# andrewcsmith/soundsym

Measured on AMD Instinct MI355X. Metric: segment-pairs/sec (DTW cost+argmin), higher is better.
Workload: dtype f32

## Files before the change

soundsym_amd/csrc/dtw_filter.hip:

```cpp
#include "ssym_internal.hpp"
#include "dtw_filter_kernel.hpp"
#include "dtw_filter_wg_kernel.hpp"
#include "dtw_filter_wg2_kernel.hpp"
#include "dtw_filter_pk_kernel.hpp"
#include "dtw_filter_sp_kernel.hpp"
#include "dtw_band_kernel.hpp"

#include <algorithm>
#include <atomic>
#include <cmath>
#include <cstdlib>

namespace ssym {

static std::atomic<unsigned long long> g_filter_wg_launches{0};
static std::atomic<unsigned long long> g_filter_wg2_launches{0};
static std::atomic<bool> g_filter_wg2{true};

int filter_pieces(int dim)
{
    static const bool k48 = ssym_knob("SSYM_FILTER_K48") != nullptr;
    return dim > kFilterMaxDim2 ? 1 : (k48 ? 2 : 3);
}

__global__ void build_filter_records_kernel(const double *__restrict__ raw, const uint64_t *__restrict__ off,
                                            const uint32_t *__restrict__ perm, uint32_t n, uint32_t dim,
                                            uint32_t dimUse, uint32_t frames_pad, int is_source,
                                            int lead, int pieces, double scale, _Float16 *__restrict__ rec,
                                            unsigned *__restrict__ resid)
{
    const uint32_t s = blockIdx.y;
    const uint32_t seg = perm[s];
    const uint32_t slot = blockIdx.x * blockDim.x + threadIdx.x;
    if (slot >= frames_pad)
        return;
    _Float16 out[kFilterRecHalfs];
#pragma unroll
    for (int i = 0; i < kFilterRecHalfs; ++i)
        out[i] = (_Float16)0.0f;
    const uint32_t nf = seg < n ? (uint32_t)(off[seg + 1] - off[seg]) : 0u;
    const uint32_t first = lead < 0 ? frames_pad - nf : (uint32_t)lead;
    const bool real = slot >= first && slot < first + nf;
    const uint32_t f = slot - first;
    const int nbase = pieces == 3 ? 28 : (pieces == 2 ? 3 : 1) * (int)dimUse;
    const int npieces = pieces == 3 ? 2 : 3;
    if (!real && is_source)
        out[filter_slot_offset(nbase)] = (_Float16)__builtin_inff();
    if (real) {
        const double *p = raw + (off[seg] + f) * dim;
        double nrm = 0.0, res2 = 0.0;
        for (uint32_t e = 0; e < dimUse; ++e) {
            const double v = p[e] * scale;
            const _Float16 h1 = (_Float16)v;
            const bool two = pieces == 2 || (pieces == 3 && (is_source || e < 2));
            const _Float16 h2 = two ? (_Float16)(v - (double)h1) : (_Float16)0.0f;
            const double vh = (double)h1 + (double)h2;
            nrm += vh * vh;
            res2 += (v - vh) * (v - vh);
            const _Float16 m1 = (_Float16)(-2.0f * (float)h1), m2 = (_Float16)(-2.0f * (float)h2);
            if (pieces == 2) {
                out[filter_slot_offset(3 * e + 0)] = is_source ? m1 : h1;
                out[filter_slot_offset(3 * e + 1)] = is_source ? m1 : h2;
                out[filter_slot_offset(3 * e + 2)] = is_source ? m2 : h1;
            } else if (pieces == 3) {
                out[filter_slot_offset(2 * e + 0)] = is_source ? m1 : h1;
                out[filter_slot_offset(2 * e + 1)] = is_source ? m2 : h1;
                if (e < 2)
                    out[filter_slot_offset(26 + e)] = is_source ? m1 : h2;
            } else {
                out[filter_slot_offset(e)] = is_source ? m1 : h1;
            }
        }
        const float r = __double2float_ru(sqrt(res2) / scale * 1.0000001);
        if (r > 0.0f)
            atomicMax(&resid[s], __float_as_uint(r));
        const _Float16 p1 = (_Float16)nrm;
        const _Float16 p2 = (_Float16)(nrm - (double)p1);
        const _Float16 p3 = (_Float16)(nrm - (double)p1 - (double)p2);
        const int mine = nbase + (is_source ? 0 : npieces), other = nbase + (is_source ? npieces : 0);
        out[filter_slot_offset(mine + 0)] = p1;
        out[filter_slot_offset(mine + 1)] = p2;
        out[filter_slot_offset(other + 0)] = (_Float16)1.0f;
        out[filter_slot_offset(other + 1)] = (_Float16)1.0f;
        if (npieces == 3) {
            out[filter_slot_offset(mine + 2)] = p3;
            out[filter_slot_offset(other + 2)] = (_Float16)1.0f;
        }
    }
    if (is_source) {
        _Float16 *dst = rec + ((size_t)s * frames_pad + slot) * kFilterRecHalfs;
#pragma unroll
        for (int i = 0; i < kFilterRecHalfs; ++i)
            dst[i] = out[i];
    } else {
#pragma unroll
        for (int h = 0; h < 2; ++h)
#pragma unroll
            for (int m = 0; m < kFilterKM; ++m) {
                _Float16 *dst = rec + tgt_rec_offset(s, frames_pad, slot, m, h);
#pragma unroll
// ... 7 lines not shown
{
    const uint32_t kb = (uint32_t)(2 * radius + 1 + 15) / 16 * 16;
    return std::max<uint32_t>(radius + src.max_frames, std::max<uint32_t>(tgt.max_frames, 1) + kb) + 1;
}
static size_t band_lds_bytes(int radius, const SegmentSet &src, const SegmentSet &tgt)
{
    return ((size_t)2 * band_slots(radius, src, tgt) * kFilterRecHalfs + kBandImagePad) * sizeof(_Float16);
}

bool filter_band_as_bound(const ssym_ctx *ctx, const SegmentSet &src, const SegmentSet &tgt)
{
    if (ctx->band < 0)
        return false;
    return 2 * ctx->band + 1 > 6 * 16 || band_lds_bytes(ctx->band, src, tgt) > 160 * 1024 - 64;
}

bool filter_supported(const ssym_ctx *ctx, const SegmentSet &src, const SegmentSet &tgt)
{
    if (src.light || tgt.light)
        return false;
    if (src.dim != tgt.dim)
        return false;
    if ((ctx->band < 0 || filter_band_as_bound(ctx, src, tgt)) && filter_shape((int)src.max_frames).nt == 0)
        return false;
    if (!std::isfinite(src.max_abs) || !std::isfinite(tgt.max_abs))
        return false;
    if (!std::isfinite(src.max_sqnorm_all) || !std::isfinite(tgt.max_sqnorm_all))
        return false;
    return src.n > 0 && tgt.n > 0;
}

static double common_scale(const SegmentSet &src, const SegmentSet &tgt)
{
    const double m = std::max(src.max_abs, tgt.max_abs);
    if (!(m > 0.0))
        return 1.0;
    int e = 0;
    (void)std::frexp(m, &e);
    e = std::min(std::max(6 - e, -100), 100);
    const double sq = std::max(src.max_sqnorm_all, tgt.max_sqnorm_all);
    while (e > -200 && sq * std::ldexp(1.0, 2 * e) * 1.01 >= 65000.0)
        --e;
    const double ideal = std::ldexp(1.0, e);
    if (src.rec && src.rec_scale > 0.0 && src.rec_scale <= ideal && src.rec_scale * 16.0 >= ideal)
        return src.rec_scale;
    return ideal;
}

static int32_t ensure_records(ssym_ctx *ctx, const SegmentSet &set, double scale, uint32_t slots, int lead)
{
    const size_t bytes = (size_t)set.n_pad * slots * kFilterRecHalfs * sizeof(_Float16);
    if (set.rec && set.rec_scale == scale && set.rec_bytes == bytes && set.rec_slots == slots &&
        set.rec_lead == lead)
        return SSYM_OK;
    if (set.rec && set.rec_bytes != bytes) {
        dev_free(ctx, set.rec);
        set.rec = nullptr;
    }
    if (!set.rec) {
        int32_t rca = dev_alloc(ctx, &set.rec, bytes);
        if (rca != SSYM_OK)
            return rca;
    }
    set.rec_bytes = bytes;
    dim3 grid((slots + 63) / 64, set.n_pad);
    const int dimUse = filter_dim_used((int)set.dim);
    unsigned *resid = (unsigned *)(set.max_sqnorm + 2 * (size_t)set.n_pad);
    SSYM_HIP_CHECK(ctx, hipMemsetAsync(resid, 0, sizeof(unsigned) * set.n_pad, ctx->stream));
    build_filter_records_kernel<<<grid, 64, 0, ctx->stream>>>(set.raw, set.off, set.perm, set.n, set.dim,
                                                              (uint32_t)dimUse, slots, set.is_source ? 1 : 0, lead,
                                                              filter_pieces(dimUse), scale,
                                                              (_Float16 *)set.rec, resid);
    SSYM_HIP_CHECK(ctx, hipGetLastError());
    set.rec_scale = scale;
    set.rec_slots = slots;
    set.rec_lead = lead;
    return SSYM_OK;
}

static FilterKnobs read_filter_knobs()
{
    FilterKnobs k;
    g_filter_wg2.store(true, std::memory_order_relaxed);
    if (!ssym_knob("SSYM_TEST_HOOKS"))
        return k;
    auto num = [](const char *name, int unset) {
        const char *v = ssym_knob(name);
        return v ? atoi(v) : unset;
    };
    k.pk = num("SSYM_FILTER_PK", 0) != 0;
    k.sp = num("SSYM_FILTER_SP", 1) != 0;
    const int mp = num("SSYM_SP_MULTIPAIR", 1);
    k.spMultipair = mp == 0 || mp == 2 ? mp : 1;
    k.spPairBlock = ssym_knob("SSYM_SP_PAIRBLOCK") ? std::max(num("SSYM_SP_PAIRBLOCK", 0), 0) : -1;
    k.wg = num("SSYM_FILTER_WG", k.wg) != 0;
    g_filter_wg2.store(num("SSYM_FILTER_WG2", 1) != 0, std::memory_order_relaxed);
    k.skip0 = num("SSYM_FILTER_SKIP0", 1) != 0;
    k.nt8 = ssym_knob("SSYM_FILTER_NT8") != nullptr;
    k.oneLaunch = ssym_knob("SSYM_FILTER_ONE_LAUNCH") != nullptr;
    k.longClasses = num("SSYM_FILTER_LONG_CLASSES", 1) != 0;
    k.pruneNt = num("SSYM_PRUNE_NT", 0);
    return k;
}

static const std::vector<uint32_t> &plan_lens(const SegmentSet &set, uint32_t group)
{
    if (set.plan_lens.size() != set.n_pad / group) {
        set.plan_lens.assign(set.n_pad / group, 0u);
        for (uint32_t slot = 0; slot < set.n; ++slot) {
            const uint32_t s = set.h_perm[slot];
            uint32_t &m = set.plan_lens[slot / group];
            m = std::max(m, (uint32_t)(set.h_off[s + 1] - set.h_off[s]));
        }
    }
    return set.plan_lens;
}

struct FilterCall {
    hipStream_t st;
    const SegmentSet &src, &tgt;
    bool sq;
    int ku;
    float outScale;
    float *handoff;
    unsigned *taskCtr;
    float *cmat;
    const float *abandon;
    unsigned long long *colCtr;
    const uint32_t *candSlot;
    bool wg2;
};

template <int NT, bool SQ, int KU>
static bool run_kernel(const FilterCall &c, const FilterLaunch &l)
{
    constexpr int OCC = NT == 1 ? 3 : NT == 8 ? 1 : 2;
    const dim3 grid(l.grid), block(64 * kFilterWavesPerBlock);
    const _Float16 *srec = (const _Float16 *)c.src.rec, *trec = (const _Float16 *)c.tgt.rec;
    const int rowsPad = (int)c.src.frames_pad, colsPad = (int)c.tgt.frames_pad, tgtPad = (int)c.tgt.n_pad;
    const int nSrcPairs = l.hi - l.lo, nTasks = nSrcPairs * (tgtPad / 32);
    unsigned *ctr = c.taskCtr + l.ctrSet * 8 * kTaskCtrStride;
    switch (l.kind) {
    case FilterKernel::Mp:
        if constexpr (NT == 1) {
            dtw_filter_sp_kernel<KU == 2 ? 3 : 2, SQ, 2, KU, kSpRowBlock, true><<<grid, block, 0, c.st>>>(
                srec, trec, c.src.len, c.tgt.len, rowsPad, colsPad, tgtPad, l.taskPairs, nSrcPairs, l.taskChunk, c.outScale,
                ctr, c.cmat, l.origin, l.lo, l.pairBlock);
            return true;
        }
        return false;
    case FilterKernel::Sp:
        if constexpr (NT <= 3 && (KU == 2 || NT <= 2)) {
            constexpr int OCCSP = (NT == 1 && KU == 2) ? 3 : (NT == 2 && KU == 2) ? SSYM_SP_OCC_NT2 : 2;
            dtw_filter_sp_kernel<NT, SQ, OCCSP, KU, kSpRowBlock><<<grid, block, 0, c.st>>>(
                srec, trec, c.src.len, c.tgt.len, rowsPad, colsPad, tgtPad, nSrcPairs, nTasks, l.taskChunk, c.outScale, ctr,
                c.cmat, l.origin, l.lo, l.pairBlock);
            return true;
        }
        return false;
    case FilterKernel::GenericSkip0:
        if constexpr (NT == 3 || NT == 4) {
            dtw_filter_kernel<NT, SQ, OCC, false, KU, true><<<grid, block, 0, c.st>>>(
                srec, trec, c.src.len, c.tgt.len, rowsPad, l.passes, colsPad, tgtPad, nSrcPairs, nTasks, l.taskChunk,
                c.outScale, c.handoff, ctr, c.cmat, nullptr, nullptr, nullptr, l.origin, l.lo);
            return true;
        }
        return false;
    case FilterKernel::Wg:
        if constexpr (NT == 4) {
            if (l.passes == 2 && c.wg2) {
                dtw_filter_wg2_kernel<SQ, KU><<<grid, block, 0, c.st>>>(
                    srec, trec, c.src.len, c.tgt.len, rowsPad, colsPad, tgtPad, nSrcPairs / 4, l.taskChunk, c.outScale, ctr,
                    c.cmat, l.origin, l.lo);
                g_filter_wg_launches.fetch_add(1, std::memory_order_relaxed);
                g_filter_wg2_launches.fetch_add(1, std::memory_order_relaxed);
                return true;
            }
            dtw_filter_wg_kernel<SQ, KU><<<grid, block, 0, c.st>>>(
                srec, trec, c.src.len, c.tgt.len, rowsPad, l.passes, colsPad, tgtPad, nSrcPairs / 4, l.taskChunk, c.outScale,
                c.handoff, ctr, c.cmat, l.origin, l.lo);
            g_filter_wg_launches.fetch_add(1, std::memory_order_relaxed);
            return true;
        }
        return false;
    case FilterKernel::Pk:
        if constexpr (NT == 4) {
            dtw_filter_pk_kernel<SQ, KU><<<grid, block, 0, c.st>>>(
                srec, trec, c.src.len, c.tgt.len, rowsPad, l.passes, colsPad, tgtPad, nSrcPairs, nTasks, l.taskChunk,
                c.outScale, c.handoff, ctr, c.cmat, l.origin, l.lo);
            return true;
        }
        return false;
    case FilterKernel::GenericPrune:
        dtw_filter_kernel<NT, SQ, OCC, true, KU><<<grid, block, 0, c.st>>>(
            srec, trec, c.src.len, c.tgt.len, rowsPad, l.passes, colsPad, tgtPad, nSrcPairs, nTasks, l.taskChunk, c.outScale,
            c.handoff, ctr, c.cmat, c.abandon, c.colCtr, c.candSlot, l.origin, l.lo);
        return true;
    case FilterKernel::Generic:
        dtw_filter_kernel<NT, SQ, OCC, false, KU><<<grid, block, 0, c.st>>>(
            srec, trec, c.src.len, c.tgt.len, rowsPad, l.passes, colsPad, tgtPad, nSrcPairs, nTasks, l.taskChunk, c.outScale,
            c.handoff, ctr, c.cmat, nullptr, nullptr, nullptr, l.origin, l.lo);
        return true;
    }
    return false;
}

template <int NT>
static bool run_tiles(const FilterCall &c, const FilterLaunch &l)
{
    if (c.sq)
        return c.ku == 2 ? run_kernel<NT, true, 2>(c, l) : run_kernel<NT, true, 3>(c, l);
    return c.ku == 2 ? run_kernel<NT, false, 2>(c, l) : run_kernel<NT, false, 3>(c, l);
}

static bool run_launch(const FilterCall &c, const FilterLaunch &l)
{
    switch (l.nt) {
    case 1: return run_tiles<1>(c, l);
    case 2: return run_tiles<2>(c, l);
    case 3: return run_tiles<3>(c, l);
    case 4: return run_tiles<4>(c, l);
    case 8: return run_tiles<8>(c, l);
    }
    return false;
}

template <int NTB, int WB, int OCC, bool SQ, int LASTN, bool PRUNE>
static int32_t launch_band_cfg2(ssym_ctx *ctx, const SegmentSet &src, const SegmentSet &tgt, uint32_t slots,
                                size_t lds, float outScale, float *cmat, const float *abandon,
                                unsigned long long *colCtr, const uint32_t *candSlot)
{
    const int nTgtBlocks = (int)tgt.n_pad / (32 * WB);
    const int nTasks = ((int)src.n_pad / 2) * nTgtBlocks;
    const int grid = std::max(1, std::min(ctx->num_cus, nTasks));
    int32_t rc = ensure(ctx, ctx->handoff, 8 * sizeof(unsigned));
    if (rc != SSYM_OK)
        return rc;
    unsigned *taskCtr = (unsigned *)ctx->handoff.ptr;
    rc = zero_words(ctx, taskCtr, sizeof(unsigned));
    if (rc != SSYM_OK)
        return rc;
    const bool two = filter_mfmas(filter_pieces(filter_dim_used((int)src.dim)), filter_dim_used((int)src.dim)) == 2;
    auto kern = two ? dtw_band_kernel<NTB, WB, OCC, SQ, LASTN, PRUNE, 2> : dtw_band_kernel<NTB, WB, OCC, SQ, LASTN, PRUNE, 3>;
#ifdef SSYM_BAND_PAIRCOLS_BUILD
    if constexpr (!PRUNE && LASTN == 1 && NTB >= 4 && OCC == 2) {
        const char *pc = ssym_knob("SSYM_BAND_PAIRCOLS");
        if (pc && atoi(pc) != 0)
            kern = two ? dtw_band_kernel<NTB, WB, OCC, SQ, LASTN, PRUNE, 2, true> : dtw_band_kernel<NTB, WB, OCC, SQ, LASTN, PRUNE, 3, true>;
    }
#endif
    if (lds > 64 * 1024)
        SSYM_HIP_CHECK(ctx, hipFuncSetAttribute((const void *)kern, hipFuncAttributeMaxDynamicSharedMemorySize, (int)lds));
    kern<<<dim3(grid), 64 * WB, lds, ctx->stream>>>(
// ... 40 lines not shown
        return rc;
    rc = ensure_records(ctx, tgt, scale, tgt.frames_pad, 0);
    if (rc != SSYM_OK)
        return rc;
    const bool sq = ctx->squared != 0;
    const float outScale = (float)(sq ? 1.0 / (scale * scale) : 1.0 / scale);
    const int ntb = (2 * ctx->band + 1 + 15) / 16;
#define SSYM_BCASE(N_)                                                                                  \
    case N_:                                                                                            \
        return sq ? launch_band<N_, true>(ctx, src, tgt, slots, lds, outScale, cmat, abandon, colCtr, candSlot)   \
                  : launch_band<N_, false>(ctx, src, tgt, slots, lds, outScale, cmat, abandon, colCtr, candSlot);
    switch (ntb) {
        SSYM_BCASE(1) SSYM_BCASE(2) SSYM_BCASE(3) SSYM_BCASE(4) SSYM_BCASE(5) SSYM_BCASE(6)
    default:
        ctx->err = "dtw band filter: band radius too large";
        return SSYM_E_UNSUPPORTED;
    }
#undef SSYM_BCASE
}

int32_t ensure_filter_records(ssym_ctx *ctx, const SegmentSet &src, const SegmentSet &tgt, double *scale_out)
{
    const double scale = common_scale(src, tgt);
    int32_t rc = ctx->band >= 0 && !filter_band_as_bound(ctx, src, tgt)
                     ? ensure_records(ctx, src, scale, band_slots(ctx->band, src, tgt), ctx->band)
                     : ensure_records(ctx, src, scale, src.frames_pad, -1);
    if (rc == SSYM_OK)
        rc = ensure_records(ctx, tgt, scale, tgt.frames_pad, 0);
    if (scale_out)
        *scale_out = scale;
    return rc;
}

int32_t launch_dtw_filter(ssym_ctx *ctx, const SegmentSet &src, const SegmentSet &tgt, float *cmat,
                          const float *abandon, unsigned long long *colCtr, const uint32_t *candSlot)
{
    ctx->filter_launches = 1;
    if (ctx->band >= 0 && !filter_band_as_bound(ctx, src, tgt))
        return launch_dtw_filter_banded(ctx, src, tgt, cmat, abandon, colCtr, candSlot);
    const FilterShape shape = filter_shape((int)src.max_frames);
    if (shape.nt == 0 || (int)src.frames_pad != shape.rows() || src.n_pad % 8 != 0 || tgt.n_pad % 32 != 0) {
        ctx->err = "dtw filter: segment set not padded for the filter kernel";
        return SSYM_E_UNSUPPORTED;
    }
    if (((size_t)tgt.frames_pad + 3) / 4 * 1024 >= ((size_t)1 << 31)) {
        ctx->err = "dtw filter: targets too long for the hand-off rows";
        return SSYM_E_UNSUPPORTED;
    }
    const double scale = common_scale(src, tgt);
    int32_t rc = ensure_records(ctx, src, scale, src.frames_pad, -1);
    if (rc != SSYM_OK)
        return rc;
    rc = ensure_records(ctx, tgt, scale, tgt.frames_pad, 0);
    if (rc != SSYM_OK)
        return rc;
    const int gridBlocks = std::max(8, ctx->num_cus * 2 / 8 * 8);
    const size_t handBytes = (size_t)(gridBlocks / 2 * 3) * kFilterWavesPerBlock * ((tgt.frames_pad + 3) / 4) * 256 * sizeof(float);
    const size_t ctrBytes = 8 * kTaskCtrStride * sizeof(unsigned);
    rc = ensure(ctx, ctx->handoff, handBytes + kMaxClasses * ctrBytes);
    if (rc != SSYM_OK)
        return rc;
    unsigned *taskCtr = (unsigned *)((char *)ctx->handoff.ptr + handBytes);
    rc = zero_words(ctx, taskCtr, kMaxClasses * ctrBytes);
    if (rc != SSYM_OK)
        return rc;
    const bool sq = ctx->squared != 0;
    const int dimUse = filter_dim_used((int)src.dim);

    FilterPlanInput in;
    in.pairLen = plan_lens(src, 2).data(), in.groupCols = plan_lens(tgt, 32).data();
    in.srcN = src.n, in.srcNPad = src.n_pad, in.framesPad = src.frames_pad;
    in.tgtN = tgt.n, in.tgtGroups = tgt.n_pad / 32, in.tgtTotalFrames = tgt.total_frames;
    in.numCus = ctx->num_cus;
    in.ku = filter_mfmas(filter_pieces(dimUse), dimUse);
    in.abandon = abandon != nullptr;
    in.pruneSwept = ctx->prune_swept;
    in.knobs = read_filter_knobs();
    const std::vector<FilterLaunch> plan = plan_filter(in);

    ctx->filter_launches = (int)plan.size();
    ctx->launched_cells = 0;
    for (const FilterLaunch &l : plan)
        ctx->launched_cells += l.cells;
    const FilterCall call{ctx->stream, src, tgt, sq, in.ku, (float)(sq ? 1.0 / (scale * scale) : 1.0 / scale),
                          (float *)ctx->handoff.ptr, taskCtr, cmat, abandon, colCtr, candSlot,
                          g_filter_wg2.load(std::memory_order_relaxed)};
    for (const FilterLaunch &l : plan)
        if (!run_launch(call, l)) {
            ctx->err = "dtw filter: the plan names a kernel that is not built";
            return SSYM_E_UNSUPPORTED;
        }
    SSYM_HIP_CHECK(ctx, hipGetLastError());
    return SSYM_OK;
}

}

extern "C" __attribute__((visibility("default"))) unsigned long long ssym_debug_filter_wg_launches(void)
{
    return ssym::g_filter_wg_launches.load(std::memory_order_relaxed);
}

extern "C" __attribute__((visibility("default"))) unsigned long long ssym_debug_filter_wg2_launches(void)
{
    return ssym::g_filter_wg2_launches.load(std::memory_order_relaxed);
}

#ifdef SSYM_SP_PROF
extern "C" __attribute__((visibility("default"))) int ssym_debug_sp_prof(unsigned long long *out)
{
    unsigned long long zero[12] = {0, 0, 0, 0, 0, 0, 0, 0, 0, 0, 0, 0};
    if (hipMemcpyFromSymbol(out, HIP_SYMBOL(ssym::ssym_sp_prof), sizeof(zero)) != hipSuccess)
        return -1;
    return hipMemcpyToSymbol(HIP_SYMBOL(ssym::ssym_sp_prof), zero, sizeof(zero)) == hipSuccess ? 0 : -1;
}
#endif
```

soundsym_amd/csrc/dtw_filter_wg2_kernel.hpp:

```cpp
#pragma once
#include "dtw_filter_kernel.hpp"

namespace ssym {

#define SSYM_FILTER_SBASE(P_) asm volatile("" : "+s"(P_))
#define SSYM_FILTER_LANEOFF(V_) asm volatile("" : "+v"(V_))

constexpr int kFilterWg2Ring = 16;
constexpr int kFilterWg2HandBytes = 2 * 2 * 1024;
constexpr int kFilterWg2RecBytes = 2 * 16;
constexpr int kFilterWg2LenBytes = 256;
constexpr int kFilterWg2Lds = kFilterWg2Ring * kFilterSlotBytes + kFilterWg2HandBytes + kFilterWg2RecBytes + kFilterWg2LenBytes;
constexpr int wait_vmcnt_lgkm0(int n) { return wait_vmcnt(n) & ~0x0F00; }

template <bool SQ, int KU>
__global__ __launch_bounds__(64 * kFilterWavesPerBlock, 2) void dtw_filter_wg2_kernel(
    const _Float16 *__restrict__ srcRec, const _Float16 *__restrict__ tgtRec,
    const int *__restrict__ srcLen, const int *__restrict__ tgtLen, int srcRows,
    int tgtFramesPad, int mPad, int nSrcBlocks, int taskChunk, float outScale,
    unsigned *__restrict__ taskCtr, float *__restrict__ cmat, int rowOrigin, int spBase)
{
    static_assert(KU == 2 || KU == 3, "two or three operand planes per column");
    static_assert(kFilterWavesPerBlock == 4, "two pairs x two roles; a column group is one column per wave");
    constexpr int NT = 4;
    constexpr int REC = kFilterRecHalfs;
    constexpr int BR = NT * 16;
    const float INF = __builtin_inff();

    const int lane = threadIdx.x & 63;
    const int wave = __builtin_amdgcn_readfirstlane(threadIdx.x >> 6);
    const int follower = wave & 1;
    const int col = lane & 31;
    const int half = lane >> 5;
    uint32_t laneOff16 = lane * 16;
    __shared__ __attribute__((aligned(16))) char lds[kFilterWg2Lds];
    char *const ring = lds;
    char *const hand = lds + kFilterWg2Ring * kFilterSlotBytes + (wave >> 1) * 2048;
    volatile int *const record = reinterpret_cast<volatile int *>(lds + kFilterWg2Ring * kFilterSlotBytes + kFilterWg2HandBytes);

    char *const lenBuf = lds + kFilterWg2Ring * kFilterSlotBytes + kFilterWg2HandBytes + kFilterWg2RecBytes;
    uint32_t laneOff4 = lane * 4;

    const unsigned nGroups = (unsigned)mPad >> 5;

    struct Item { int tg, sp0, nCols, g; };
    Item im1{0, 0, 0, -1}, i0{0, 0, 0, -1}, i1{0, 0, 0, -1}, i2{0, 0, 0, -1};
    unsigned hop = 0;
    unsigned requests = 0;
    bool pending = false;
    bool request = false;
    unsigned tick = 0;
    unsigned feGi = 0, feEnd = 0, feHalf = 0, feXcd = 0, feRange = 0;
    bool feOn = false, feAtomic = false, feValid = false;
    unsigned feTk = 0;
    int feTg = 0, feSp0 = 0;

    auto last_group = [](const Item &it) __attribute__((always_inline)) { return 4 * (it.g + 1) >= it.nCols; };

    auto open_tick = [&](bool storeYoungest) __attribute__((always_inline)) -> bool {
        if (storeYoungest)
            __builtin_amdgcn_s_waitcnt(wait_vmcnt_lgkm0(1));
        else
            __builtin_amdgcn_s_waitcnt(wait_vmcnt_lgkm0(0));
        asm volatile("" ::: "memory");
        __builtin_amdgcn_s_barrier();
        asm volatile("" ::: "memory");
        im1 = i0;
        i0 = i1;
        i1 = i2;
        if (i2.g >= 0 && !last_group(i2)) {
            ++i2.g;
        } else if (pending) {
            const unsigned slot = (requests - 1u) & 1u;
            const int tg = __builtin_amdgcn_readfirstlane(record[4 * slot + 0]);
            const int sp0 = __builtin_amdgcn_readfirstlane(record[4 * slot + 1]);
            const int nc = __builtin_amdgcn_readfirstlane(record[4 * slot + 2]);
            if (tg >= 0) {
                i2 = Item{tg, sp0, nc, 0};
            } else {
                i2.g = -1;
                ++hop;
            }
        } else {
            i2.g = -1;
        }
        pending = false;
        if (hop >= 8u && im1.g < 0 && i0.g < 0 && i1.g < 0 && i2.g < 0)
            return false;
        request = hop < 8u && (i2.g < 0 || last_group(i2));
        if (request) {
            pending = true;
            ++requests;
        }
        feOn = request && wave == 0;
        if (feOn) {
            feXcd = (blockIdx.x + hop) & 7u;
            feRange = feXcd < nGroups ? ((nGroups - feXcd + 7u) >> 3) * (unsigned)nSrcBlocks : 0u;
            feAtomic = feGi >= feEnd;
            if (feAtomic && lane == 0)
                feTk = atomicAdd(&taskCtr[feXcd * kTaskCtrStride], (unsigned)taskChunk);
        }
        if (i2.g >= 0) {
            const int cc = max(min(4 * i2.g + wave, i2.nCols - 1), 0);
            char *slot = ring + ((4 * (tick + 2u) + (unsigned)wave) & (unsigned)(kFilterWg2Ring - 1)) * kFilterSlotBytes;
            const char *gb = reinterpret_cast<const char *>(tgtRec) +
                             ((size_t)(unsigned)i2.tg * (unsigned)tgtFramesPad + (unsigned)cc) * (kTgtFrameHalfs * 2);
// ... 94 lines not shown
    };

    if (!follower) {
        float up = INF;
        asm volatile("" : "+v"(up));
        for (;; ++tick) {
            if (!open_tick(false))
                break;
            if (i0.g >= 0) {
                const unsigned vg = tick & 3u;
                if (i0.g == 0)
                    start_task(i0, rowOrigin, vg);
                char *const handW = hand + (tick & 1u) * 1024 + lane * 4;
                auto column = [&](int q) __attribute__((always_inline)) {
                    const float diag = prevTop;
                    prevTop = up;
                    float bottom;
                    if ((q & 1) == 0) {
                        fetch(4u * vg + q + 1, B1);
                        bottom = dp_column<NT, SQ, KU>(A, B0, B1, acc, up, diag, L0, L1);
                    } else {
                        fetch(4u * vg + q + 1, B0);
                        bottom = dp_column<NT, SQ, KU>(A, B1, B0, acc, up, diag, L1, L0);
                    }
                    *reinterpret_cast<float *>(handW + q * 256) = bottom;
                };
                column(0);
                column(1);
                front_end_task();
                column(2);
                column(3);
                front_end_record();
            } else {
                front_end_task();
                front_end_record();
            }
        }
    } else {
        float res = INF;
        int fb_m1 = -1;
        bool stored = false;
        for (;; ++tick) {
            if (!open_tick(stored))
                break;
            stored = false;
            if (im1.g >= 0) {
                const unsigned vg = (tick + 3u) & 3u;
                const char *const handR = hand + ((tick + 1u) & 1u) * 1024 + lane * 4;
                float topN = *reinterpret_cast<const float *>(handR);
                if (im1.g == 0) {
                    fb_m1 = tgtLen[32 * im1.tg + col] - 1;
                    res = INF;
                    start_task(im1, rowOrigin + BR, vg);
                }
                const int j0 = 4 * im1.g;
                auto column = [&](int q) __attribute__((always_inline)) {
                    const float up = topN;
                    const float diag = prevTop;
                    prevTop = up;
                    if (q < 3)
                        topN = *reinterpret_cast<const float *>(handR + (q + 1) * 256);
                    float bottom;
                    if ((q & 1) == 0) {
                        fetch(4u * vg + q + 1, B1);
                        bottom = dp_column<NT, SQ, KU>(A, B0, B1, acc, up, diag, L0, L1);
                    } else {
                        fetch(4u * vg + q + 1, B0);
                        bottom = dp_column<NT, SQ, KU>(A, B1, B0, acc, up, diag, L1, L0);
                    }
                    res = (j0 + q == fb_m1) ? bottom : res;
                };
                column(0);
                column(1);
                column(2);
                column(3);
                if (last_group(im1)) {
                    const int sp = im1.sp0 + (wave >> 1);
                    cmat[(size_t)(2 * sp + half) * mPad + 32 * im1.tg + col] = res * outScale;
                    stored = true;
                }
            }
        }
    }
}

#undef SSYM_FILTER_SBASE
#undef SSYM_FILTER_LANEOFF

}
```

soundsym_amd/csrc/pack.hip:

```cpp
#include "ssym_internal.hpp"

#include <algorithm>
#include <cstring>

namespace ssym {

int32_t ensure(ssym_ctx *ctx, DeviceBuf &b, size_t bytes)
{
    if (bytes <= b.bytes && b.ptr)
        return SSYM_OK;
    if (b.ptr && ctx->stream_only) {
        ctx->deferred_free.push_back(b.ptr);
        b.ptr = nullptr;
        b.bytes = 0;
    }
    if (b.ptr) {
        SSYM_HIP_CHECK(ctx, hipStreamSynchronize(ctx->stream));
        SSYM_HIP_CHECK(ctx, hipFree(b.ptr));
        b.ptr = nullptr;
        b.bytes = 0;
    }
    size_t want = std::max<size_t>(bytes, 256);
    SSYM_HIP_CHECK(ctx, hipMalloc(&b.ptr, want));
    b.bytes = want;
// ... 169 lines not shown

char *stage_take(ssym_ctx *ctx, size_t bytes)
{
    if (bytes > kStageMaxCopy)
        return nullptr;
    if (!ctx->stage) {
        if (hipHostMalloc((void **)&ctx->stage, kStageBytes, hipHostMallocDefault) != hipSuccess) {
            (void)hipGetLastError();
            ctx->stage = nullptr;
            return nullptr;
        }
        ctx->stage_cap = kStageBytes;
    }
    const size_t at = (ctx->stage_cur + 63) & ~(size_t)63;
    if (at + bytes > ctx->stage_cap)
        return nullptr;
    ctx->stage_cur = at + bytes;
    return ctx->stage + at;
}

int32_t stage_h2d(ssym_ctx *ctx, void *dst_dev, const void *src_host, size_t bytes)
{
    if (bytes == 0)
        return SSYM_OK;
    char *p = ctx->api_depth > 0 ? stage_take(ctx, bytes) : nullptr;
    if (p) {
        memcpy(p, src_host, bytes);
        src_host = p;
    }
    SSYM_HIP_CHECK(ctx, hipMemcpyAsync(dst_dev, src_host, bytes, hipMemcpyHostToDevice, ctx->stream));
    return SSYM_OK;
}

int32_t stage_d2h(ssym_ctx *ctx, void *dst_host, const void *src_dev, size_t bytes)
{
    if (bytes == 0)
        return SSYM_OK;
    char *p = ctx->api_depth > 0 ? stage_take(ctx, bytes) : nullptr;
    if (p) {
        SSYM_HIP_CHECK(ctx, hipMemcpyAsync(p, src_dev, bytes, hipMemcpyDeviceToHost, ctx->stream));
        ctx->pending_d2h.push_back({dst_host, p, bytes});
        return SSYM_OK;
    }
    SSYM_HIP_CHECK(ctx, hipMemcpyAsync(dst_host, src_dev, bytes, hipMemcpyDeviceToHost, ctx->stream));
    return SSYM_OK;
}

void stage_finish(ssym_ctx *ctx)
{
    for (const auto &d : ctx->pending_d2h)
        memcpy(d.user, d.pinned, d.bytes);
    ctx->pending_d2h.clear();
}

void free_segments(ssym_ctx *ctx, SegmentSet &set)
{
    dev_free(ctx, set.raw);
    dev_free(ctx, set.off);
    dev_free(ctx, set.norm);
    dev_free(ctx, set.rec);
    set.rec = nullptr;
    dev_free(ctx, set.len);
    dev_free(ctx, set.max_sqnorm);
    dev_free(ctx, set.perm);
    dev_free(ctx, set.centroid);
    dev_free(ctx, set.len_order);
    refcos_q8_release(ctx, set);
    set = SegmentSet{};
}

static int32_t build_derived(ssym_ctx *ctx, SegmentSet &set)
{
    hipStream_t st = ctx->stream;
    const uint32_t n = set.n, dim = set.dim;
    dev_free(ctx, set.off); set.off = nullptr;
    dev_free(ctx, set.norm); set.norm = nullptr;
    dev_free(ctx, set.len); set.len = nullptr;
    dev_free(ctx, set.max_sqnorm); set.max_sqnorm = nullptr;
    dev_free(ctx, set.perm); set.perm = nullptr;
    dev_free(ctx, set.centroid); set.centroid = nullptr; set.centroid_n = 0;
    dev_free(ctx, set.len_order); set.len_order = nullptr; set.len_order_n = 0;
    refcos_q8_release(ctx, set);
    set.plan_lens.clear();

    set.max_frames = 0;
    for (uint32_t i = 0; i < n; ++i)
        set.max_frames = std::max<uint32_t>(set.max_frames, (uint32_t)(set.h_off[i + 1] - set.h_off[i]));

    { int32_t rca = dev_alloc(ctx, (void **)&set.off, sizeof(uint64_t) * (n + 1)); if (rca != SSYM_OK) return rca; }
    { int32_t rcs = stage_h2d(ctx, set.off, set.h_off.data(), sizeof(uint64_t) * (n + 1)); if (rcs != SSYM_OK) return rcs; }
    if (n == 0) {
        SSYM_HIP_CHECK(ctx, hipStreamSynchronize(st));
        return SSYM_OK;
    }

    if (ctx->metric == SSYM_METRIC_REFCOS) {
        { int32_t rca = dev_alloc(ctx, (void **)&set.norm, sizeof(double) * 3 * (size_t)n); if (rca != SSYM_OK) return rca; }
        segment_norm_kernel<<<(n + 3) / 4, 256, 0, st>>>(set.raw, set.off, n, dim, set.norm);
        SSYM_HIP_CHECK(ctx, hipGetLastError());
    } else if (ctx->pack_light && !set.is_source) {
        set.light = true;
    } else {
        const uint32_t quantum = (!set.is_source && ctx->band >= 0) ? 256u : 32u;
        set.n_pad = (n + quantum - 1) / quantum * quantum;
        uint32_t mf = std::max<uint32_t>(set.max_frames, 1);
        FilterShape shape = filter_shape((int)mf);
        set.frames_pad = set.is_source ? (shape.nt ? (uint32_t)shape.rows() : mf) : mf;
        set.h_perm.assign(set.n_pad, 0xffffffffu);
        for (uint32_t i = 0; i < n; ++i)
            set.h_perm[i] = i;
        std::stable_sort(set.h_perm.begin(), set.h_perm.begin() + n, [&](uint32_t a, uint32_t b) {
            return set.h_off[a + 1] - set.h_off[a] < set.h_off[b + 1] - set.h_off[b];
        });
        { int32_t rca = dev_alloc(ctx, (void **)&set.perm, sizeof(uint32_t) * set.n_pad); if (rca != SSYM_OK) return rca; }
        { int32_t rcs = stage_h2d(ctx, set.perm, set.h_perm.data(), sizeof(uint32_t) * set.n_pad); if (rcs != SSYM_OK) return rcs; }
        constexpr size_t kLenTailPad = 8;
        { int32_t rca = dev_alloc(ctx, (void **)&set.len, sizeof(int32_t) * (set.n_pad + kLenTailPad)); if (rca != SSYM_OK) return rca; }
        SSYM_HIP_CHECK(ctx, hipMemsetAsync(set.len, 0, sizeof(int32_t) * (set.n_pad + kLenTailPad), st));
        { int32_t rca = dev_alloc(ctx, (void **)&set.max_sqnorm, sizeof(float) * 3 * (size_t)set.n_pad); if (rca != SSYM_OK) return rca; }
        SSYM_HIP_CHECK(ctx, hipMemsetAsync(set.max_sqnorm, 0, sizeof(float) * 3 * (size_t)set.n_pad, st));
        dim3 grid((mf + 63) / 64, n);
        segment_stats_kernel<<<grid, 64, 0, st>>>(set.raw, set.off, set.perm, n, dim, set.len,
                                                  (unsigned *)set.max_sqnorm,
                                                  (unsigned *)set.max_sqnorm + set.n_pad);
        SSYM_HIP_CHECK(ctx, hipGetLastError());
        std::vector<float> h(2 * (size_t)set.n_pad);
        SSYM_HIP_CHECK(ctx, hipMemcpyAsync(h.data(), set.max_sqnorm, sizeof(float) * 2 * (size_t)set.n_pad,
                                           hipMemcpyDeviceToHost, st));
        SSYM_HIP_CHECK(ctx, hipStreamSynchronize(st));
        float m = 0.f, ma = 0.f;
        for (uint32_t i = 0; i < set.n_pad; ++i) {
            m = std::max(m, h[i]);
            ma = std::max(ma, h[set.n_pad + i]);
        }
        set.max_sqnorm_all = (double)m;
        set.max_abs = (double)ma;
        dev_free(ctx, set.rec);
        set.rec = nullptr;
        set.rec_scale = 0.0;
        set.rec_bytes = 0;
    }
    if (!ctx->defer_sync)
        SSYM_HIP_CHECK(ctx, hipStreamSynchronize(st));
    return SSYM_OK;
}

static int32_t validate_offsets(ssym_ctx *ctx, const uint64_t *off, uint32_t n)
{
    if (!off) {
        ctx->err = "frame_offsets is NULL";
        return SSYM_E_INVALID;
    }
    for (uint32_t i = 0; i < n; ++i) {
        if (off[i + 1] < off[i]) {
            ctx->err = "frame_offsets must be non-decreasing";
            return SSYM_E_INVALID;
        }
        if (off[i + 1] - off[i] > 0x7fffffffull) {
            ctx->err = "segment too long";
            return SSYM_E_INVALID;
        }
    }
    return SSYM_OK;
}

static int32_t upload_values(ssym_ctx *ctx, SegmentSet &set, size_t dst_val_offset, const void *feats,
// ... 123 lines not shown
```

soundsym_amd/csrc/ssym_internal.hpp:

```cpp
#pragma once

#include <hip/hip_runtime.h>

#include <cstdint>
#include <cstdlib>
#include <exception>
#include <map>
#include <new>
#include <string>
#include <unordered_map>
#include <vector>

#include "soundsym_amd.h"
#include "dtw_filter_plan.hpp"

inline const char *ssym_knob(const char *name)
{
    const char *h = getenv("SSYM_TEST_HOOKS");
    return (h && atoi(h) != 0) ? getenv(name) : nullptr;
}

namespace ssym {


int filter_pieces(int dim);

constexpr size_t kRawTailPad = 2;

struct DeviceBuf {
    void *ptr = nullptr;
    size_t bytes = 0;
};

struct SegmentSet {
    double *raw = nullptr;
    uint64_t *off = nullptr;
    std::vector<uint64_t> h_off;
    uint32_t n = 0;
    uint32_t dim = 0;
    uint64_t total_frames = 0;
    uint32_t max_frames = 0;
    double *norm = nullptr;
    int32_t *len = nullptr;
    float *max_sqnorm = nullptr;
    double max_sqnorm_all = 0.0;
    double max_abs = 0.0;
    uint32_t n_pad = 0;
    uint32_t frames_pad = 0;
    bool is_source = false;
    bool light = false;
    mutable void *rec = nullptr;
    mutable double rec_scale = 0.0;
    uint32_t *perm = nullptr;
    std::vector<uint32_t> h_perm;
    mutable std::vector<uint32_t> plan_lens;
    mutable size_t rec_bytes = 0;
    mutable uint32_t rec_slots = 0;
    mutable int rec_lead = 0;
    size_t raw_capacity_vals = 0;
    mutable float *centroid = nullptr;
    mutable uint32_t centroid_n = 0;
    mutable uint32_t *len_order = nullptr;
    mutable uint32_t len_order_n = 0;
    mutable int8_t *q8 = nullptr;
    mutable double *q8_info = nullptr;
    mutable uint32_t q8_rows = 0;
    mutable uint32_t q8_groups = 0;
    mutable int q8_state = 0;
};

}

struct ssym_ctx {
    int device = 0;
    int metric = SSYM_METRIC_DTW;
    int dtype = SSYM_DTYPE_F32;
    int band = -1;
    int squared = 0;
    bool prune_default = false;
    hipStream_t stream = nullptr;
    bool owns_stream = false;
    std::string err;
    ssym_timings timings{};
    int num_cus = 256;
    ssym::DeviceBuf handoff;
    ssym::DeviceBuf cmat;
    ssym::DeviceBuf tmin;
    ssym::DeviceBuf tmin2;
    ssym::DeviceBuf cand;
    ssym::DeviceBuf selmask;
    ssym::DeviceBuf selcnt;
    ssym::DeviceBuf cand2;
    ssym::DeviceBuf cand_xmin;
    ssym::DeviceBuf cand_cost;
    ssym::DeviceBuf best;
    ssym::DeviceBuf topk;
    ssym::DeviceBuf prune_pairs, prune_cost;
    ssym::DeviceBuf abandon;
    ssym::DeviceBuf dist;
    ssym::DeviceBuf part;
    ssym::DeviceBuf paced_part;
    ssym::DeviceBuf cover_tab;
    ssym::DeviceBuf mosaic_tab;
    ssym::DeviceBuf one_ticket;
    ssym::DeviceBuf out_idx, out_cost;
    ssym::DeviceBuf zeros;
    ssym::DeviceBuf stamps;
    double wall_clock_khz = 0;
    ssym::DeviceBuf pipe_flag;
    int pipe_slot = 0;
    unsigned pipe_mask = 0;
    hipEvent_t ev[10]{};
    float prune_swept = 1.f;
    unsigned long long pruned_cells = 0;
    int filter_launches = 1;
    unsigned long long launched_cells = 0;
    bool defer_sync = false;
    bool pack_light = false;
    bool stream_only = false;
    std::vector<void *> deferred_free;
    uint64_t so_cap = 0;
    const uint32_t *so_hdr1 = nullptr, *so_hdr2 = nullptr;
    bool so_filter = false;
    bool so_refcos = false;
    struct Pending {
        bool valid = false, filter = false, has_dist = false;
        bool cand = false;
        bool pruned = false;
        const ssym_dict *dict = nullptr;
        const ssym_queries *q = nullptr;
        uint32_t index_base = 0;
        std::vector<double> dist_host;
        float main_ms = 0.f;
    } pending;
    char *stage = nullptr;
    size_t stage_cap = 0, stage_cur = 0;
    int api_depth = 0;
    struct PendingD2H { void *user; const void *pinned; size_t bytes; };
// ... 276 lines not shown
```

Baseline: 527.3 million.

## Add uniform-length specialization of wg2 DTW filter kernel

Adds a templated UNIFORM path to the two-pass workgroup DTW filter kernel, used when every target segment (and the source pairs in a launch) has the same frame count. With lengths known uniform, the kernel walks only uniF/4 column groups per task and stores the final column directly, dropping per-lane length masking and per-task length lookups. The host records per-group minimum lengths to detect uniformity. This adds a large duplicated kernel body and only fires when the shape conditions hold.

```diff
diff --git a/soundsym_amd/csrc/dtw_filter.hip b/soundsym_amd/csrc/dtw_filter.hip
--- a/soundsym_amd/csrc/dtw_filter.hip
+++ b/soundsym_amd/csrc/dtw_filter.hip
@@ -16,6 +16,8 @@
 static std::atomic<unsigned long long> g_filter_wg_launches{0};
 static std::atomic<unsigned long long> g_filter_wg2_launches{0};
 static std::atomic<bool> g_filter_wg2{true};
+static std::atomic<unsigned long long> g_filter_wg2u_launches{0};
+static std::atomic<bool> g_filter_wg2u{true};
 
 int filter_pieces(int dim)
 {
@@ -189,6 +191,7 @@
 {
     FilterKnobs k;
     g_filter_wg2.store(true, std::memory_order_relaxed);
+    g_filter_wg2u.store(true, std::memory_order_relaxed);
     if (!ssym_knob("SSYM_TEST_HOOKS"))
         return k;
     auto num = [](const char *name, int unset) {
@@ -202,6 +205,7 @@
     k.spPairBlock = ssym_knob("SSYM_SP_PAIRBLOCK") ? std::max(num("SSYM_SP_PAIRBLOCK", 0), 0) : -1;
     k.wg = num("SSYM_FILTER_WG", k.wg) != 0;
     g_filter_wg2.store(num("SSYM_FILTER_WG2", 1) != 0, std::memory_order_relaxed);
+    g_filter_wg2u.store(num("SSYM_FILTER_WG2U", 1) != 0, std::memory_order_relaxed);
     k.skip0 = num("SSYM_FILTER_SKIP0", 1) != 0;
     k.nt8 = ssym_knob("SSYM_FILTER_NT8") != nullptr;
     k.oneLaunch = ssym_knob("SSYM_FILTER_ONE_LAUNCH") != nullptr;
@@ -214,13 +218,24 @@
 {
     if (set.plan_lens.size() != set.n_pad / group) {
         set.plan_lens.assign(set.n_pad / group, 0u);
+        set.plan_min_lens.assign(set.n_pad / group, 0xffffffffu);
         for (uint32_t slot = 0; slot < set.n; ++slot) {
             const uint32_t s = set.h_perm[slot];
-            uint32_t &m = set.plan_lens[slot / group];
-            m = std::max(m, (uint32_t)(set.h_off[s + 1] - set.h_off[s]));
+            const uint32_t f = (uint32_t)(set.h_off[s + 1] - set.h_off[s]);
+            uint32_t &m = set.plan_lens[slot / group], &lo = set.plan_min_lens[slot / group];
+            m = std::max(m, f);
+            lo = std::min(lo, f);
         }
     }
     return set.plan_lens;
+}
+
+static uint32_t uniform_len(const SegmentSet &set, uint32_t group, uint32_t lo, uint32_t hi)
+{
+    const std::vector<uint32_t> &longest = plan_lens(set, group);
+    if (lo >= hi || hi > longest.size() || (uint64_t)hi * group > set.n)
+        return 0;
+    return set.plan_min_lens[lo] == longest[hi - 1] ? longest[hi - 1] : 0;
 }
 
 struct FilterCall {
@@ -236,6 +251,7 @@
     unsigned long long *colCtr;
     const uint32_t *candSlot;
     bool wg2;
+    uint32_t uniF;
 };
 
 template <int NT, bool SQ, int KU>
@@ -276,6 +292,16 @@
     case FilterKernel::Wg:
         if constexpr (NT == 4) {
             if (l.passes == 2 && c.wg2) {
+                const uint32_t uniFa = c.uniF && rowsPad - l.origin == 128 ? uniform_len(c.src, 2, l.lo, l.hi) : 0;
+                if (uniFa > 64 && uniFa <= 128) {
+                    dtw_filter_wg2_kernel<SQ, KU, true><<<grid, block, 0, c.st>>>(
+                        srec, trec, c.src.len, c.tgt.len, rowsPad, colsPad, tgtPad, nSrcPairs / 4, l.taskChunk, c.outScale, ctr,
+                        c.cmat, l.origin, l.lo, (int)c.uniF, (int)uniFa);
+                    g_filter_wg_launches.fetch_add(1, std::memory_order_relaxed);
+                    g_filter_wg2_launches.fetch_add(1, std::memory_order_relaxed);
+                    g_filter_wg2u_launches.fetch_add(1, std::memory_order_relaxed);
+                    return true;
+                }
                 dtw_filter_wg2_kernel<SQ, KU><<<grid, block, 0, c.st>>>(
                     srec, trec, c.src.len, c.tgt.len, rowsPad, colsPad, tgtPad, nSrcPairs / 4, l.taskChunk, c.outScale, ctr,
                     c.cmat, l.origin, l.lo);
@@ -482,9 +508,13 @@
     ctx->launched_cells = 0;
     for (const FilterLaunch &l : plan)
         ctx->launched_cells += l.cells;
+    uint32_t uniF = g_filter_wg2u.load(std::memory_order_relaxed) && !abandon && tgt.n == tgt.n_pad
+                        ? uniform_len(tgt, 32, 0, tgt.n_pad / 32) : 0;
+    if (uniF < 4 || uniF % 4 != 0 || uniF > tgt.frames_pad)
+        uniF = 0;
     const FilterCall call{ctx->stream, src, tgt, sq, in.ku, (float)(sq ? 1.0 / (scale * scale) : 1.0 / scale),
                           (float *)ctx->handoff.ptr, taskCtr, cmat, abandon, colCtr, candSlot,
-                          g_filter_wg2.load(std::memory_order_relaxed)};
+                          g_filter_wg2.load(std::memory_order_relaxed), uniF};
     for (const FilterLaunch &l : plan)
         if (!run_launch(call, l)) {
             ctx->err = "dtw filter: the plan names a kernel that is not built";
@@ -506,6 +536,11 @@
     return ssym::g_filter_wg2_launches.load(std::memory_order_relaxed);
 }
 
+extern "C" __attribute__((visibility("default"))) unsigned long long ssym_debug_filter_wg2u_launches(void)
+{
+    return ssym::g_filter_wg2u_launches.load(std::memory_order_relaxed);
+}
+
 #ifdef SSYM_SP_PROF
 extern "C" __attribute__((visibility("default"))) int ssym_debug_sp_prof(unsigned long long *out)
 {
diff --git a/soundsym_amd/csrc/dtw_filter_wg2_kernel.hpp b/soundsym_amd/csrc/dtw_filter_wg2_kernel.hpp
--- a/soundsym_amd/csrc/dtw_filter_wg2_kernel.hpp
+++ b/soundsym_amd/csrc/dtw_filter_wg2_kernel.hpp
@@ -13,15 +13,280 @@
 constexpr int kFilterWg2Lds = kFilterWg2Ring * kFilterSlotBytes + kFilterWg2HandBytes + kFilterWg2RecBytes + kFilterWg2LenBytes;
 constexpr int wait_vmcnt_lgkm0(int n) { return wait_vmcnt(n) & ~0x0F00; }
 
-template <bool SQ, int KU>
+template <int NT, bool SQ, int KU>
+__device__ __forceinline__ float dp_column_first(const half8 (&A)[NT][KU], const half8 (&Bc)[KU], const half8 (&Bn)[KU],
+                                                 f32x16 &acc, float up, float (&Lw)[NT * 16])
+{
+#pragma unroll
+    for (int T = 0; T < NT; ++T) {
+        f32x16 accn;
+        if (T + 1 < NT)
+            accn = mfma_tile<KU>(A[T + 1], Bc);
+        else
+            accn = mfma_tile<KU>(A[0], Bn);
+#pragma unroll
+        for (int r = 0; r < 16; ++r) {
+            const float x = acc[r];
+            const float c = SQ ? __builtin_fabsf(x) : __builtin_amdgcn_sqrtf(__builtin_fabsf(x));
+            const float cur = c + up;
+            Lw[T * 16 + r] = cur;
+            up = cur;
+        }
+        acc = accn;
+    }
+    return up;
+}
+
+template <bool SQ, int KU, bool UNIFORM = false>
 __global__ __launch_bounds__(64 * kFilterWavesPerBlock, 2) void dtw_filter_wg2_kernel(
     const _Float16 *__restrict__ srcRec, const _Float16 *__restrict__ tgtRec,
     const int *__restrict__ srcLen, const int *__restrict__ tgtLen, int srcRows,
     int tgtFramesPad, int mPad, int nSrcBlocks, int taskChunk, float outScale,
-    unsigned *__restrict__ taskCtr, float *__restrict__ cmat, int rowOrigin, int spBase)
+    unsigned *__restrict__ taskCtr, float *__restrict__ cmat, int rowOrigin, int spBase, int uniF = 0, int uniFa = 0)
 {
     static_assert(KU == 2 || KU == 3, "two or three operand planes per column");
     static_assert(kFilterWavesPerBlock == 4, "two pairs x two roles; a column group is one column per wave");
+   if constexpr (UNIFORM) {
+    constexpr int NT = 4;
+    constexpr int REC = kFilterRecHalfs;
+    constexpr int BR = NT * 16;
+    const float INF = __builtin_inff();
+
+    const int lane = threadIdx.x & 63;
+    const int wave = __builtin_amdgcn_readfirstlane(threadIdx.x >> 6);
+    const int follower = wave & 1;
+    const int col = lane & 31;
+    const int half = lane >> 5;
+    uint32_t laneOff16 = lane * 16;
+    __shared__ __attribute__((aligned(16))) char lds[kFilterWg2Lds - kFilterWg2LenBytes];
+    char *const ring = lds;
+    char *const hand = lds + kFilterWg2Ring * kFilterSlotBytes + (wave >> 1) * 2048;
+    volatile int *const record = reinterpret_cast<volatile int *>(lds + kFilterWg2Ring * kFilterSlotBytes + kFilterWg2HandBytes);
+
+    const unsigned nGroups = (unsigned)mPad >> 5;
+    const int lastG = (uniF >> 2) - 1;
+
+    struct Item { int tg, sp0, g; };
+    Item im1{0, 0, -1}, i0{0, 0, -1}, i1{0, 0, -1}, i2{0, 0, -1};
+    unsigned hop = 0;
+    unsigned requests = 0;
+    bool pending = false;
+    bool request = false;
+    unsigned tick = 0;
+    unsigned feGi = 0, feEnd = 0, feHalf = 0, feXcd = 0, feRange = 0;
+    bool feOn = false, feAtomic = false;
+    unsigned feTk = 0;
+
+    auto open_tick = [&](bool storeYoungest) __attribute__((always_inline)) -> bool {
+        if (storeYoungest)
+            __builtin_amdgcn_s_waitcnt(wait_vmcnt_lgkm0(1));
+        else
+            __builtin_amdgcn_s_waitcnt(wait_vmcnt_lgkm0(0));
+        asm volatile("" ::: "memory");
+        __builtin_amdgcn_s_barrier();
+        asm volatile("" ::: "memory");
+        im1 = i0;
+        i0 = i1;
+        i1 = i2;
+        if (i2.g >= 0 && i2.g != lastG) {
+            ++i2.g;
+        } else if (pending) {
+            const unsigned slot = (requests - 1u) & 1u;
+            const int tg = __builtin_amdgcn_readfirstlane(record[4 * slot + 0]);
+            const int sp0 = __builtin_amdgcn_readfirstlane(record[4 * slot + 1]);
+            if (tg >= 0) {
+                i2 = Item{tg, sp0, 0};
+            } else {
+                i2.g = -1;
+                ++hop;
+            }
+        } else {
+            i2.g = -1;
+        }
+        pending = false;
+        if (hop >= 8u && (im1.g & i0.g & i1.g & i2.g) < 0)
+            return false;
+        request = hop < 8u && (i2.g < 0 || i2.g == lastG);
+        if (request) {
+            pending = true;
+            ++requests;
+        }
+        feOn = request && wave == 0;
+        if (feOn) {
+            feXcd = (blockIdx.x + hop) & 7u;
+            feRange = feXcd < nGroups ? ((nGroups - feXcd + 7u) >> 3) * (unsigned)nSrcBlocks : 0u;
+            feAtomic = feGi >= feEnd;
+            if (feAtomic && lane == 0)
+                feTk = atomicAdd(&taskCtr[feXcd * kTaskCtrStride], (unsigned)taskChunk);
+        }
+        if (i2.g >= 0) {
+            const int cc = 4 * i2.g + wave;
+            char *slot = ring + ((4 * (tick + 2u) + (unsigned)wave) & (unsigned)(kFilterWg2Ring - 1)) * kFilterSlotBytes;
+            const char *gb = reinterpret_cast<const char *>(tgtRec) +
+                             ((size_t)(unsigned)i2.tg * (unsigned)tgtFramesPad + (unsigned)cc) * (kTgtFrameHalfs * 2);
+            SSYM_FILTER_SBASE(gb);
+            SSYM_FILTER_LANEOFF(laneOff16);
+            const __attribute__((address_space(1))) void *gp =
+                (const __attribute__((address_space(1))) void *)(gb + laneOff16);
+            __attribute__((address_space(3))) void *lp = (__attribute__((address_space(3))) void *)slot;
+            __builtin_amdgcn_global_load_lds(gp, lp, 16, 0, 0);
+            __builtin_amdgcn_global_load_lds(gp, lp, 16, 1024, 0);
+            if (KU == 3)
+                __builtin_amdgcn_global_load_lds(gp, lp, 16, 2048, 0);
+        }
+        asm volatile("" ::: "memory");
+        return true;
+    };
+    auto front_end = [&]() __attribute__((always_inline)) {
+        if (feOn) {
+            if (feAtomic) {
+                feGi = (unsigned)__builtin_amdgcn_readfirstlane((int)feTk);
+                feEnd = min(feGi + (unsigned)taskChunk, feRange);
+                feHalf = 0;
+            }
+            int tg = -1, sp0 = 0;
+            if (feGi < feEnd) {
+                const unsigned lin = feRange - 1u - feGi;
+                tg = (int)(feXcd + 8u * (lin / (unsigned)nSrcBlocks));
+                sp0 = spBase + 4 * (int)(lin % (unsigned)nSrcBlocks) + 2 * (int)feHalf;
+                feHalf ^= 1u;
+                if (feHalf == 0)
+                    ++feGi;
+            } else {
+                feGi = feEnd = feHalf = 0;
+            }
+            const unsigned slot = (requests - 1u) & 1u;
+            if (lane == 0) {
+                record[4 * slot + 0] = tg;
+                record[4 * slot + 1] = sp0;
+            }
+        }
+    };
+    auto fetch = [&](unsigned s, half8 (&B)[KU]) __attribute__((always_inline)) {
+        const char *slot = ring + (s & (unsigned)(kFilterWg2Ring - 1)) * kFilterSlotBytes;
+#pragma unroll
+        for (int m = 0; m < KU; ++m)
+            B[m] = *reinterpret_cast<const half8 *>(slot + m * 1024 + lane * 16);
+    };
+
+    half8 A[NT][KU];
+    float L0[BR], L1[BR];
+    half8 B0[KU], B1[KU];
+    f32x16 acc;
+    float prevTop = INF;
+    auto start_task = [&](const Item &it, int rowBase, unsigned vg) __attribute__((always_inline)) {
+        const int sp = it.sp0 + (wave >> 1);
+        int ln = lane;
+        asm volatile("" : "+v"(ln));
+        const int arow = ln & 31;
+        const int a_src = 2 * sp + ((arow >> 2) & 1);
+        const int a_frm = rowBase + (arow & 3) + 4 * (arow >> 3);
+        const _Float16 *abase = srcRec + ((size_t)a_src * srcRows + a_frm) * REC + (ln >> 5) * 24;
+#pragma unroll
+        for (int T = 0; T < NT; ++T)
+            load_rec<KU>(abase + (size_t)T * kFilterRowsPerTile * REC, A[T]);
+        fetch(4u * vg, B0);
+        acc = mfma_tile<KU>(A[0], B0);
+    };
+
+    if (!follower) {
+        float up = INF;
+        asm volatile("" : "+v"(up));
+        const int zeroRow = srcRows - uniFa - 1 - rowOrigin;
+        for (;; ++tick) {
+            if (!open_tick(false))
+                break;
+            if (i0.g >= 0) {
+                const unsigned vg = tick & 3u;
+                char *const handW = hand + (tick & 1u) * 1024 + lane * 4;
+                auto column = [&](int q) __attribute__((always_inline)) {
+                    const float diag = prevTop;
+                    prevTop = up;
+                    float bottom;
+                    if ((q & 1) == 0) {
+                        fetch(4u * vg + q + 1, B1);
+                        bottom = dp_column<NT, SQ, KU>(A, B0, B1, acc, up, diag, L0, L1);
+                    } else {
+                        fetch(4u * vg + q + 1, B0);
+                        bottom = dp_column<NT, SQ, KU>(A, B1, B0, acc, up, diag, L1, L0);
+                    }
+                    *reinterpret_cast<float *>(handW + q * 256) = bottom;
+                };
+                if (i0.g == 0) {
+                    start_task(i0, rowOrigin, vg);
+                    prevTop = INF;
+                    if (zeroRow >= 0) {
+                        int z = zeroRow;
+                        asm volatile("" : "+s"(z));
+#pragma unroll
+                        for (int i = 0; i < BR; ++i) {
+                            L0[i] = (i == z) ? 0.0f : INF;
+                            L1[i] = L0[i];
+                        }
+                        column(0);
+                    } else {
+                        fetch(4u * vg + 1, B1);
+                        const float bottom = dp_column_first<NT, SQ, KU>(A, B0, B1, acc, 0.0f, L1);
+                        *reinterpret_cast<float *>(handW) = bottom;
+                    }
+                } else {
+                    column(0);
+                }
+                column(1);
+                front_end();
+                column(2);
+                column(3);
+            } else {
+                front_end();
+            }
+        }
+    } else {
+        bool stored = false;
+        for (;; ++tick) {
+            if (!open_tick(stored))
+                break;
+            stored = false;
+            if (im1.g >= 0) {
+                const unsigned vg = (tick + 3u) & 3u;
+                const char *const handR = hand + ((tick + 1u) & 1u) * 1024 + lane * 4;
+                float topN = *reinterpret_cast<const float *>(handR);
+                float bottom = INF;
+                auto column = [&](int q) __attribute__((always_inline)) {
+                    const float up = topN;
+                    const float diag = prevTop;
+                    prevTop = up;
+                    if (q < 3)
+                        topN = *reinterpret_cast<const float *>(handR + (q + 1) * 256);
+                    if ((q & 1) == 0) {
+                        fetch(4u * vg + q + 1, B1);
+                        bottom = dp_column<NT, SQ, KU>(A, B0, B1, acc, up, diag, L0, L1);
+                    } else {
+                        fetch(4u * vg + q + 1, B0);
+                        bottom = dp_column<NT, SQ, KU>(A, B1, B0, acc, up, diag, L1, L0);
+                    }
+                };
+                if (im1.g == 0) {
+                    start_task(im1, rowOrigin + BR, vg);
+                    const float up = topN;
+                    prevTop = up;
+                    topN = *reinterpret_cast<const float *>(handR + 256);
+                    fetch(4u * vg + 1, B1);
+                    bottom = dp_column_first<NT, SQ, KU>(A, B0, B1, acc, up, L1);
+                } else {
+                    column(0);
+                }
+                column(1);
+                column(2);
+                column(3);
+                if (im1.g == lastG) {
+                    const int sp = im1.sp0 + (wave >> 1);
+                    cmat[(size_t)(2 * sp + half) * mPad + 32 * im1.tg + col] = bottom * outScale;
+                    stored = true;
+                }
+            }
+        }
+    }
+   } else {
     constexpr int NT = 4;
     constexpr int REC = kFilterRecHalfs;
     constexpr int BR = NT * 16;
@@ -282,6 +547,7 @@
             }
         }
     }
+   }
 }
 
 #undef SSYM_FILTER_SBASE
diff --git a/soundsym_amd/csrc/pack.hip b/soundsym_amd/csrc/pack.hip
--- a/soundsym_amd/csrc/pack.hip
+++ b/soundsym_amd/csrc/pack.hip
@@ -275,6 +275,7 @@
     dev_free(ctx, set.len_order); set.len_order = nullptr; set.len_order_n = 0;
     refcos_q8_release(ctx, set);
     set.plan_lens.clear();
+    set.plan_min_lens.clear();
 
     set.max_frames = 0;
     for (uint32_t i = 0; i < n; ++i)
diff --git a/soundsym_amd/csrc/ssym_internal.hpp b/soundsym_amd/csrc/ssym_internal.hpp
--- a/soundsym_amd/csrc/ssym_internal.hpp
+++ b/soundsym_amd/csrc/ssym_internal.hpp
@@ -54,6 +54,7 @@
     uint32_t *perm = nullptr;
     std::vector<uint32_t> h_perm;
     mutable std::vector<uint32_t> plan_lens;
+    mutable std::vector<uint32_t> plan_min_lens;
     mutable size_t rec_bytes = 0;
     mutable uint32_t rec_slots = 0;
     mutable int rec_lead = 0;
```

Result: faster. 532.9 million (median of 6 runs) (+1.1%).
